# tommybazar/TBRaymarcherPlugin

Hardware: AMD Instinct MI355X
Metric: volume Msamples/s (rays x steps) at 512^3, 1024^2 view; % HBM roofline (higher is better)
Workload: dtype f32

## Files before the change

tbraymarcherplugin_amd/csrc/tbrm_api.cpp:

```cpp
#include "tbrm_resources.h"
#include "tbrm_light_sweep.h"

#include <algorithm>
#include <atomic>
#include <cctype>
#include <cmath>
#include <cstdarg>
#include <cstdio>
#include <climits>
#include <cstdlib>
#include <cstring>
#include <new>
#include <vector>

using namespace tbrm;
using namespace tbrm_host;

namespace {
thread_local char g_error[512] = "";

struct TunableDef { const char* name; int def; };
const TunableDef kTunables[TUNE_COUNT] = {
    {"force_slice_kernel", 0}, {"chunk_steps", 0}, {"occ_slices", 0}, {"sparse_occ", 1}, {"occ_list", 1}, {"light_cache_mb", -1},
    {"light_batching", 1}, {"share_grid", 1}, {"ray_wave_skip", -1}, {"ray_lanes", 0}, {"chain_fast_loop", 1},
    {"chain_rect_planes", 1}, {"occ_overlap", 2}, {"light_sweep", 1}, {"sweep_prefetch", 0}, {"stream_priority", 0}, {"sweep_debug", 0},
    {"sweep_timeout_ms", 0}, {"fast_window_div", 1}, {"slab_sweep", 0}, {"gpu_timing", 1}, {"ray_tables", 1}, {"sweep_epoch_preset", 0}, {"occ_dual", 1}, {"sweep_chain", 4}, {"ray_xcd_rows", 1},
    {"ray_labels", 0}, {"stats_groups", 0}, {"occ_run", 4}, {"view_cache_mb", 1536},
};
struct TunableStore {
    std::atomic<int> v[TUNE_COUNT];
    TunableStore()
    {
        for (int t = 0; t < TUNE_COUNT; ++t) {
            char env[64] = "TBRM_";
            size_t n = strlen(env);
            for (const char* c = kTunables[t].name; *c && n + 1 < sizeof(env); ++c) env[n++] = (char) toupper((unsigned char) *c);
            env[n] = 0;
            const char* e = getenv(env);
            v[t].store(e && *e ? atoi(e) : kTunables[t].def, std::memory_order_relaxed);
        }
    }
};
TunableStore g_tunables;
}

namespace tbrm {
int tune(Tunable t) { return g_tunables.v[t].load(std::memory_order_relaxed); }
}

int tbrm_set_tunable(const char* name, int32_t value)
{
    if (!name) return tbrm_host::fail(TBRM_ERR_INVALID_ARG, "null argument");
    for (int t = 0; t < TUNE_COUNT; ++t)
        if (!strcmp(name, kTunables[t].name)) { g_tunables.v[t].store(value, std::memory_order_relaxed); return TBRM_OK; }
    return tbrm_host::fail(TBRM_ERR_INVALID_ARG, "no tunable named '%s'", name);
}

int tbrm_get_tunable(const char* name, int32_t* value)
{
    if (!name || !value) return tbrm_host::fail(TBRM_ERR_INVALID_ARG, "null argument");
    for (int t = 0; t < TUNE_COUNT; ++t)
        if (!strcmp(name, kTunables[t].name)) { *value = tune((Tunable) t); return TBRM_OK; }
    return tbrm_host::fail(TBRM_ERR_INVALID_ARG, "no tunable named '%s'", name);
}

namespace tbrm_host {

int fail(int code, const char* fmt, ...)
{
    va_list ap;
    va_start(ap, fmt);
    vsnprintf(g_error, sizeof(g_error), fmt, ap);
    va_end(ap);
    return code;
}

int bind(const tbrm_resources* r)
{
    HIP_TRY(hipSetDevice(r->desc.device));
    return TBRM_OK;
}

bool initialized(const tbrm_resources* r) { return r && r->has_volume && r->has_tf && r->d_light; }

VolumeDev data_view(const tbrm_resources* r)
{
    const tbrm_resources::Residency& q = r->res_data;
    return VolumeDev{r->d_data, r->desc.dim_x, r->desc.dim_y, r->desc.dim_z, r->desc.data_format, r->dbn[0], r->dbn[0] * r->dbn[1],
                     q.wrap_src, (q.hi - q.wrap_src) * 8};
}
static void window_division(float center, float width, float* inv_width, int* fast_div)
{
    *inv_width = 0.0f;
    *fast_div = 0;
    if (tune(TUNE_FAST_WINDOW_DIV) == 0 || !std::isfinite(center) || !std::isfinite(width)) return;
    const float aw = std::fabs(width), ac = std::fabs(center);
    if (!(aw >= 0x1p-40f && aw <= 0x1p40f) || ac > 0x1p40f) return;
    uint32_t bits;
    memcpy(&bits, &width, 4);
    if ((bits & 0x007fffffu) == 0x007fffffu) return;
    *inv_width = 1.0f / width;
    *fast_div = 1;
}

WindowDev window_dev_of(float center, float width, int low_cutoff, int high_cutoff)
{
    WindowDev w{center, width, low_cutoff ? 1.0f : 0.0f, high_cutoff ? 1.0f : 0.0f, 0.0f, 0};
    window_division(center, width, &w.inv_width, &w.fast_div);
    return w;
}
// ... 750 lines not shown
```

tbraymarcherplugin_amd/csrc/tbrm_api_render.cpp:

```cpp
#include "tbrm_resources.h"
#include "../../include/tbrm_view_cache.h"

#include <algorithm>
#include <cmath>
#include <cstdio>
#include <cstring>
#include <vector>

using namespace tbrm;
using namespace tbrm_host;

namespace {

int build_ray_params(tbrm_resources* r, const tbrm_camera* cam, const tbrm_tile* tile, const tbrm_raymarch_params* rp,
                     const tbrm_world_params* world, RayParams& p)
{
    if (!(rp->steps > 0.0f)) return fail(TBRM_ERR_INVALID_ARG, "steps must be > 0");
    if (tile->w < 0 || tile->h < 0 || cam->width <= 0 || cam->height <= 0) return fail(TBRM_ERR_INVALID_ARG, "bad tile/camera size");
    std::memset(&p, 0, sizeof(p));
    p.data = data_view(r);
    p.data_addr_mode = r->desc.data_address_mode == TBRM_ADDRESS_CLAMP ? ADDR_CLAMP : ADDR_WRAP;
    p.tf = r->d_tf;
    p.win = window_dev(r);
    p.xcd_rows = tune(TUNE_RAY_XCD_ROWS);
    p.light = r->d_light;
    for (int c = 0; c < 3; ++c) p.lv_dims[c] = r->lv_dims[c];
    p.lv_bnx = r->lbn[0];
    p.lv_bnxy = r->lbn[0] * r->lbn[1];
    p.lv_fmt = r->lv_fmt;
    p.lv_wrap_layer = r->res_light.wrap_src;
    p.lv_wrap_shift = (r->res_light.hi - r->res_light.wrap_src) * 8;
    const tbrm_vec3d* v[4] = {&cam->position, &cam->forward, &cam->right, &cam->up};
    float* dst[4] = {p.cam_pos, p.fwd, p.right, p.up};
    for (int k = 0; k < 4; ++k) {
        dst[k][0] = (float) v[k]->x; dst[k][1] = (float) v[k]->y; dst[k][2] = (float) v[k]->z;
    }
    p.thx = (float) cam->tan_half_fov_x;
    p.thy = (float) cam->tan_half_fov_y;
    p.width = cam->width;
    p.height = cam->height;
    host_world_to_local(world->volume_transform, p.m);
    host_local_clipping(*world, p.cc, p.cd);
    p.clip_mode = raymarch_clip_mode(p.cc, p.cd);
    {
        const int ws = tune(TUNE_RAY_WAVE_SKIP);
        p.wave_skip = ws > 0 || (ws < 0 && std::min(r->desc.dim_x, std::min(r->desc.dim_y, r->desc.dim_z)) >= 384) ? 1 : 0;
    }
    p.share_grid = (r->lv_dims[0] == r->desc.dim_x && r->lv_dims[1] == r->desc.dim_y && r->lv_dims[2] == r->desc.dim_z &&
                    !r->resident && tune(TUNE_SHARE_GRID)) ? 1 : 0;
    p.tile_x0 = tile->x0; p.tile_y0 = tile->y0; p.tile_w = tile->w; p.tile_h = tile->h;
    p.row_group_step = tile->row_group_step > 0 ? tile->row_group_step : 1;
    p.steps = rp->steps;
    p.jitter_frame = rp->jitter_frame;
    p.bnx = r->bn[0]; p.bny = r->bn[1]; p.bnz = r->bn[2];
    p.tab = r->d_ray_tab;
    return TBRM_OK;
}

int attach_skipping(tbrm_resources* r, const tbrm_raymarch_params* rp, RayParams& p)
{
    if (!rp->enable_skipping) return TBRM_OK;
    if (int e = ensure_skipping(r)) return e;
    p.empty_bits = r->d_empty;
    p.skip_dist = r->d_dist[0];
    return TBRM_OK;
}

template <class March> int deliver_frame(tbrm_resources* r, const tbrm_tile* tile, float* host_out_rgba, March&& march, bool* delivered = nullptr)
{
    if (!r || !tile || !host_out_rgba) return fail(TBRM_ERR_INVALID_ARG, "null argument");
    if (tile->w < 0 || tile->h < 0) return fail(TBRM_ERR_INVALID_ARG, "bad tile size");
    const size_t bytes = (size_t) tile->w * tile->h * 4 * sizeof(float);
    if (bytes == 0) return TBRM_OK;
    if (int e = bind(r)) return e;
    if (bytes > r->out_bytes) {
        HIP_TRY(hipStreamSynchronize(r->stream));
        (void) hipFree(r->d_out);
        r->d_out = nullptr;
        r->out_bytes = 0;
        HIP_TRY(hipMalloc((void**) &r->d_out, bytes));
        r->out_bytes = bytes;
    }
    if (int e = march(r->d_out)) return e;
    HIP_TRY(hipMemcpyAsync(host_out_rgba, r->d_out, bytes, hipMemcpyDeviceToHost, r->stream));
    HIP_TRY(hipStreamSynchronize(r->stream));
    if (delivered) *delivered = true;
    return TBRM_OK;
}


bool carve_view_arena(ViewCache& v, const RayParams& p)
{
    const size_t bw = 8, bh = v.lanes == 4 ? 8 : 4;
    const size_t waves = ((size_t) p.tile_w + bw - 1) / bw * (((size_t) p.tile_h + bh - 1) / bh) * 4;
    const size_t align = 256, header = (2 * waves * sizeof(uint32_t) + 16 + align - 1) / align * align;
    if (!v.arena || waves > 0xffffffffu || header + 2 * align + kRayRecordTripBytes > v.arena_bytes) return false;
    const size_t cap = std::min<size_t>((v.arena_bytes - header - align) / kRayRecordTripBytes, 0xffffffffu);
    v.n_waves = (uint32_t) waves;
    v.cap_trips = (uint32_t) cap;
    v.rec.counts = reinterpret_cast<uint32_t*>(v.arena);
    v.rec.offsets = v.rec.counts + waves;
    v.rec.meta = v.rec.offsets + waves;
    v.rec.base = reinterpret_cast<int32_t*>(v.arena + header);
    v.rec.rows = v.arena + header + (cap * sizeof(int32_t) + align - 1) / align * align;
    return true;
}

int march_or_relight(tbrm_resources* r, RayParams& p)
{
    ViewCache& v = r->view;
    const auto plain = [&]() -> int {
        HIP_TRY(launch_raymarch(p, r->stream));
        ++v.stats[0];
        return TBRM_OK;
    };
    if (tune(TUNE_VIEW_CACHE_MB) <= 0 || p.depth || r->d_labels || p.slab_on || r->resident || p.tile_w <= 0 || p.tile_h <= 0) {
        v.state = ViewCache::kNone;
        v.stats[5] = 0;
        return plain();
    }
    RayParams key;
    std::memcpy(&key, &p, sizeof(key));
    key.out = nullptr;
    const int lanes = ray_lanes_for(p), tables = ray_tables_for(p) ? 1 : 0;
    if (v.state == ViewCache::kNone || v.lanes != lanes || v.tables != tables || v.data_gen != r->data_gen || v.tf_gen != r->tf_gen ||
        std::memcmp(&v.key, &key, sizeof(key)) != 0) {
        std::memcpy(&v.key, &key, sizeof(key));
        v.lanes = lanes;
        v.tables = tables;
        v.data_gen = r->data_gen;
        v.tf_gen = r->tf_gen;
        v.state = ViewCache::kPlain;
        v.stats[5] = 0;
        return plain();
    }
    switch (v.state) {
    case ViewCache::kPlain:
        ensure_view_arena(r, false);
        if (!carve_view_arena(v, p)) {
            v.state = ViewCache::kTooLarge;
            ++v.stats[4];
            return plain();
        }
        p.rec = v.rec;
        HIP_TRY(launch_raymarch_recording(p, false, r->stream));
        v.state = ViewCache::kCounted;
        ++v.stats[1];
        return TBRM_OK;
    case ViewCache::kCounted:
        p.rec = v.rec;
        HIP_TRY(launch_view_scan(v.rec, v.n_waves, v.cap_trips, r->stream));
        HIP_TRY(launch_raymarch_recording(p, true, r->stream));
        HIP_TRY(hipMemcpyAsync(v.meta_host, v.rec.meta, 2 * sizeof(uint32_t), hipMemcpyDeviceToHost, r->stream));
        HIP_TRY(hipEventRecord(v.ev_meta, r->stream));
        v.state = ViewCache::kFilled;
        ++v.stats[2];
        return TBRM_OK;
    case ViewCache::kFilled: {
        const hipError_t q = hipEventQuery(v.ev_meta);
        if (q == hipErrorNotReady) {
            (void) hipGetLastError();
            return plain();
        }
        HIP_TRY(q);
        if (!v.meta_host[1]) {
            v.state = ViewCache::kTooLarge;
            ++v.stats[4];
            return plain();
        }
        v.state = ViewCache::kReady;
        v.stats[5] = (uint64_t) v.meta_host[0] * kRayRecordTripBytes + 2 * (uint64_t) v.n_waves * sizeof(uint32_t);
        [[fallthrough]];
    }
    case ViewCache::kReady:
        p.rec = v.rec;
        HIP_TRY(launch_relight(p, r->stream));
        ++v.stats[3];
        return TBRM_OK;
    default:
        return plain();
    }
}

}

namespace tbrm_host {

void ensure_view_arena(tbrm_resources* r, bool eager)
{
    ViewCache& v = r->view;
    const int mb = tune(TUNE_VIEW_CACHE_MB);
    if (v.arena_tried || mb <= 0 || r->resident || r->light_channels != 1) return;
    v.arena_tried = true;
    size_t want = (size_t) mb << 20, free_b = 0, total_b = 0;
    if (hipMemGetInfo(&free_b, &total_b) == hipSuccess) {
        const size_t spare = free_b > ((size_t) 8 << 30) ? free_b - ((size_t) 8 << 30) : 0;
        want = std::min(want, eager ? spare / 2 : spare / 8);
    } else (void) hipGetLastError();
    void* a = nullptr;
    void* h = nullptr;
    hipEvent_t ev = nullptr;
    if (want >= ((size_t) 64 << 10) && hipMalloc(&a, want) == hipSuccess && hipHostMalloc(&h, 4 * sizeof(uint32_t), hipHostMallocDefault) == hipSuccess &&
        hipEventCreateWithFlags(&ev, hipEventDisableTiming) == hipSuccess) {
        v.arena = (char*) a;
        v.arena_bytes = want;
        v.meta_host = (uint32_t*) h;
        v.ev_meta = ev;
        return;
    }
    (void) hipGetLastError();
    if (a) (void) hipFree(a);
    if (h) (void) hipHostFree(h);
}

void release_view_cache(tbrm_resources* r)
{
    ViewCache& v = r->view;
    if (v.arena) (void) hipFree(v.arena);
    if (v.meta_host) (void) hipHostFree(v.meta_host);
    if (v.ev_meta) (void) hipEventDestroy(v.ev_meta);
    v = ViewCache{};
}

}

extern "C" {

int tbrm_view_cache_abi_version(void) { return TBRM_VIEW_CACHE_ABI_VERSION; }

int tbrm_view_cache_stats(const tbrm_resources* r, uint64_t out[6])
{
    if (!r || !out) return fail(TBRM_ERR_INVALID_ARG, "null argument");
    for (int k = 0; k < 6; ++k) out[k] = r->view.stats[k];
    return TBRM_OK;
}

int tbrm_raymarch_lit_device(tbrm_resources* r, const tbrm_camera* cam, const tbrm_tile* tile, const tbrm_raymarch_params* rp,
                             const tbrm_world_params* world, const float* device_scene_depth, float* device_out_rgba)
{
    if (r && r->resident) return fail(TBRM_ERR_UNSUPPORTED, "slab-resident handle: frames are marched with tbrm_raymarch_lit_slab_device");
    if (!r || !cam || !tile || !rp || !world || !device_out_rgba) return fail(TBRM_ERR_INVALID_ARG, "null argument");
    if (!initialized(r)) return fail(TBRM_ERR_NOT_INITIALIZED, "resources have no volume or transfer function");
    if (int e = bind(r)) return e;
    RayParams p;
    if (int e = build_ray_params(r, cam, tile, rp, world, p)) return e;
    p.depth = device_scene_depth;
    p.out = device_out_rgba;
    if (int e = attach_skipping(r, rp, p)) return e;
    if (int e = label_ray_params(r, p)) return e;
    if (int e = begin_timed(r, 1)) return e;
    if (r->light_channels == 3) {
        p.light = r->light_channel(0);
        p.light_g = r->light_channel(1);
        p.light_b = r->light_channel(2);
        HIP_TRY(launch_raymarch_rgb(p, r->stream));
    } else if (int e = march_or_relight(r, p)) return e;
    ++r->launches[2];
    return end_timed(r, 1);
}
// ... 151 lines not shown
```

tbraymarcherplugin_amd/csrc/tbrm_internal.h:

```cpp
#pragma once
#include <hip/hip_runtime.h>
#include <stdint.h>

namespace tbrm {

enum : int { FMT_U8 = 0, FMT_U16 = 1, FMT_F32 = 2 };
enum : int { ADDR_WRAP = 0, ADDR_CLAMP = 1, ADDR_BORDER = 2 };

enum : int { PASS_ADD = 0, PASS_CHANGE = 1, PASS_ADD2 = 2, PASS_CHANGE_ONE = 3, PASS_PLANES = 5 };

constexpr int kBrick = 8;
constexpr int kBrickShift = 3;

struct VolumeDev {
    const void* data;
    int nx, ny, nz;
    int fmt;
    int bnx;
    int bnxy;
    int wrap_layer;
    int wrap_shift;
};

struct WindowDev {
// ... 75 lines not shown
    const uint8_t* occ_flags;
    int occ_phase;
    uint8_t* occ_flags_out;
    int occ_blocks_x, occ_blocks_y, occ_groups;
    int pass_start, pass_slices, chunk_slices;
    const uint32_t* occ_list;
    const int* occ_count;
    int occ_grid_cap;
    uint32_t* occ_list_out;
    int* occ_count_out;
    int* occ_count_host;
    int32_t* occ_slot_out;
    int compact;
    const float* ones;
    ChunkStream a, r;
};

struct DualPass {
    int axis, start, dir;
    int blocks_x, blocks_y;
    float step100[2];
    float* fs_keep[2];
    float* fs_spill[2];
    uint32_t fs_cap[2];
    const int32_t* fs_slot;
    const uint8_t* flags;
};
struct DualOcc {
    int on;
    DualPass pass[2];
};
constexpr int kOccRunMax = 64;
constexpr int kRunLenShift = 26;
constexpr uint32_t kRunNone = 0xffffffffu;
constexpr size_t kRunMaskWords = 4096;
struct OccRuns {
    int len;
    uint32_t* list;
    int* count;
    int* count_host;
};
struct SweepParams {
    int sx, sy;
    int hx, hy;
    int r_from_records;
    int r_sx, r_sy, r_hx, r_hy;
    uint32_t r_epoch;
    uint32_t* rec[2];
    uint32_t epoch;
    int unused0;
    int stagger_ns;
    int* ticket;
    int debug;
    unsigned long long* stamps;
    int unused1;
    int lv_f32;
    int reinit_slice;
    int n_real;
    int* error;
    unsigned long long give_up_ticks;
};

struct SweepLink {
    uint32_t* prog_out;
    const uint32_t* prog_in;
    uint32_t in_epoch;
    int in_axis, in_tiles_x;
    int in_down, in_layer0, in_G;
    int coherent_loads;
    int ticket0;
    int total_tiles;
};
constexpr int kSweepChainMax = 4;
struct SweepChainPass {
    ChunkParams p;
    SweepParams q;
    SweepLink link;
};
struct SweepChainArgs {
    int n;
    SweepChainPass pass[kSweepChainMax];
};

constexpr size_t kRayRecordRowBytes = 64 * (sizeof(float4) + 3 * sizeof(float));
constexpr size_t kRayRecordTripBytes = kRayRecordRowBytes + sizeof(int32_t);
struct RayRecord {
    uint32_t* counts;
    uint32_t* offsets;
    uint32_t* meta;
    int32_t* base;
    char* rows;
};

struct RayParams {
    VolumeDev data;
    int data_addr_mode;
    const float4* tf;
    WindowDev win;
    const void* light;
    int lv_dims[3];
    int lv_bnx, lv_bnxy;
    int lv_fmt;
    float cam_pos[3], fwd[3], right[3], up[3];
    float thx, thy;
    int width, height;
    float m[12];
    float cc[3], cd[3];
    int clip_mode;
    int share_grid;
    int wave_skip;
    int tile_x0, tile_y0, tile_w, tile_h, row_group_step;
    float steps;
    int jitter_frame;
    const float* depth;
    float* out;
    const uint32_t* empty_bits;
    int xcd_rows;
    const uint2* tab;
    const uint8_t* skip_dist;
    int bnx, bny, bnz;
    unsigned long long* sample_counter;
    int lv_wrap_layer, lv_wrap_shift;
    int slab_on, slab_z0, slab_z1, slab_dir;
    const uint16_t* octree;
    int oct_dims[3];
    float oct_depth0;
    const uint8_t* labels;
    const float4* lab_colors;
    const void* light_g;
    const void* light_b;
    RayRecord rec;
};

int ray_lanes_for(const RayParams& p);
bool ray_tables_for(const RayParams& p);

constexpr int kRayTabApron = 2;
constexpr int ray_tab_axis_entries(int n) { return n + 2 * kRayTabApron; }
constexpr int ray_tab_index(int texel) { return texel + kRayTabApron; }
constexpr int ray_tab_last_base(int n) { return ray_tab_axis_entries(n) - 2; }
constexpr int ray_tab_entries(int nx, int ny, int nz) { return (ray_tab_axis_entries(nx) + ray_tab_axis_entries(ny) + ray_tab_axis_entries(nz) + 1) & ~1; }

struct BrickParams {
    VolumeDev data;
    int addr_mode;
    int bnx, bny, bnz;
    float2* minmax;
    int bz0, bz1;
};

struct EmptyParams {
    const float2* minmax;
    int n_bricks;
    WindowDev win;
    const int* alpha_prefix;
    uint32_t* bits;
};

hipError_t launch_shell_transparent(const EmptyParams& p, int bnx, int bny, int bnz, float border, int* flag, hipStream_t s);

constexpr int kSkipDistCap = 32;
struct DistParams {
    const uint32_t* bits;
    const uint8_t* in;
    uint8_t* out;
    int bn[3];
    int axis;
};

struct OctreeParams {
    VolumeDev data;
    const uint16_t* lower;
    int lower_dims[3];
    uint16_t* out;
    int dims[3];
};

struct RelayoutParams {
    const void* src;
    void* dst;
    int nx, ny, nz;
    int bnx, bnxy, bnz;
    int elem_bytes;
    int to_bricks;
};

constexpr int kOccSlices = 8;
constexpr int kChunkTile = 32;
constexpr int kChunkThreads = 1024;
constexpr int kChunkMaxHull = 64;

enum Tunable : int {
    TUNE_FORCE_SLICE_KERNEL,
    TUNE_CHUNK_STEPS,
    TUNE_OCC_SLICES,
    TUNE_SPARSE_OCC,
    TUNE_OCC_LIST,
    TUNE_LIGHT_CACHE_MB,
    TUNE_LIGHT_BATCHING,
    TUNE_SHARE_GRID,
    TUNE_RAY_WAVE_SKIP,
    TUNE_RAY_LANES,
    TUNE_CHAIN_FAST_LOOP,
    TUNE_CHAIN_RECT_PLANES,
    TUNE_OCC_OVERLAP,
    TUNE_LIGHT_SWEEP,
    TUNE_SWEEP_PREFETCH,
    TUNE_STREAM_PRIORITY,
    TUNE_SWEEP_DEBUG,
    TUNE_SWEEP_TIMEOUT_MS,
    TUNE_FAST_WINDOW_DIV,
    TUNE_SLAB_SWEEP,
    TUNE_GPU_TIMING,
    TUNE_RAY_TABLES,
    TUNE_SWEEP_EPOCH_PRESET,
    TUNE_OCC_DUAL,
    TUNE_SWEEP_CHAIN,
    TUNE_RAY_XCD_ROWS,
    TUNE_RAY_LABELS,
    TUNE_STATS_GROUPS,
    TUNE_OCC_RUN,
    TUNE_VIEW_CACHE_MB,
    TUNE_COUNT
};
int tune(Tunable t);

hipError_t launch_selftest_decode(float* d_u8, float* d_u16, hipStream_t s);
hipError_t launch_selftest_roundtrip(const float* d_in, float* d_out, size_t n, hipStream_t s);
hipError_t launch_selftest_window_division(const WindowDev& w, unsigned long long* d_mismatches, hipStream_t s);
hipError_t launch_selftest_opacity_correction(float step0, float step1, unsigned long long* d_mismatches, hipStream_t s);
hipError_t launch_relayout(const RelayoutParams& p, hipStream_t s);
size_t chunk_lds_bytes(const ChunkParams& p, int mode, int lv_fmt);
size_t occlusion_lds_bytes(const ChunkParams& p);
constexpr int kPlaneGuard = 4096;
hipError_t launch_occ_flags(const ChunkParams& p, int mode, int n_chunks, hipStream_t s);
hipError_t launch_light_occlusion(const ChunkParams& p, int mode, hipStream_t s, const DualOcc* dual = nullptr, const OccRuns* runs = nullptr);
hipError_t launch_unit_flags(const ChunkParams& pc, const DualOcc& d, hipStream_t s);
bool occ_runs_apply(const ChunkParams& pc);
hipError_t launch_occ_runs(const ChunkParams& pc, const OccRuns& runs, hipStream_t s);
hipError_t launch_light_chain(const ChunkParams& p, int mode, int lv_fmt, hipStream_t s);
hipError_t launch_light_sweep(const ChunkParams& p, const SweepParams& q, int mode, hipStream_t s);
hipError_t launch_light_sweep_chain(const SweepChainArgs& c, int mode, hipStream_t s);
hipError_t launch_fill(void* dst, int fmt, size_t n, float value, hipStream_t s);
hipError_t launch_propagate_slice(const PropParams& p, bool change, hipStream_t s);
hipError_t launch_raymarch(const RayParams& p, hipStream_t s);
hipError_t launch_raymarch_rgb(const RayParams& p, hipStream_t s);
hipError_t launch_raymarch_recording(const RayParams& p, bool fill, hipStream_t s);
hipError_t launch_view_scan(const RayRecord& rec, uint32_t n_waves, uint32_t cap_trips, hipStream_t s);
hipError_t launch_relight(const RayParams& p, hipStream_t s);
hipError_t launch_raymarch_intensity(const RayParams& p, hipStream_t s);
hipError_t launch_raymarch_octree(const RayParams& p, hipStream_t s);
hipError_t launch_octree_level(const OctreeParams& p, bool base, hipStream_t s);
hipError_t launch_count_samples(const RayParams& p, hipStream_t s);
hipError_t launch_brick_minmax(const BrickParams& p, hipStream_t s);
hipError_t launch_brick_empty(const EmptyParams& p, hipStream_t s);
hipError_t launch_brick_dist(const DistParams& p, int addr_mode, hipStream_t s);

struct LabelBrickParams {
    const uint8_t* labels;
    uint32_t* masks;
    int bnx, bny;
    int b0[3], b1[3];
};
struct LabelLiveParams {
    const uint32_t* masks;
    int n_bricks;
    uint32_t alive[8];
    uint32_t* live;
    uint32_t* present;
};
struct LabelMergeParams {
    const uint32_t* empty;
    const uint32_t* live;
    uint32_t* out;
    int bn[3];
};
struct LabelRegionParams {
    const uint8_t* src;
    uint8_t* dst;
    int origin[3], extent[3];
    int bnx, bnxy;
};
hipError_t launch_label_brick_masks(const LabelBrickParams& p, hipStream_t s);
hipError_t launch_label_live(const LabelLiveParams& p, hipStream_t s);
hipError_t launch_label_merge(const LabelMergeParams& p, int addr_mode, hipStream_t s);
hipError_t launch_label_region(const LabelRegionParams& p, hipStream_t s);

struct VolumeRegionParams {
    const void* box;
    void* bricked;
    int origin[3], extent[3];
    int bnx, bnxy;
    int elem_bytes;
    int to_bricks;
};
struct BrickReach {
    int lo[3], hi[3], last[3];
    int n[3];
};
hipError_t launch_volume_region(const VolumeRegionParams& p, hipStream_t s);
hipError_t launch_brick_minmax_region(const BrickParams& p, const BrickReach& q, hipStream_t s);

constexpr int kStatsMaxBins = 4096;
constexpr int kStatsLabelWords = 256 * 6;
struct StatsParams {
    const void* data;
    const uint8_t* labels;
    int fmt;
    int bnx, bnxy;
    int origin[3], end[3];
    int b0[3], nb[3];
    uint32_t n_bins;
    uint32_t lo_code, hi_code;
    uint32_t div_mul, div_shift;
    float lo_f, hi_f, scale;
    uint32_t copies;
    uint32_t mask[8];
    uint32_t* out;
};
hipError_t launch_volume_histogram(const StatsParams& p, bool masked, int grid, hipStream_t s);
hipError_t launch_label_statistics(const StatsParams& p, int grid, hipStream_t s);

}
```

tbraymarcherplugin_amd/csrc/tbrm_kernels.hip:

```cpp
#include "tbrm_device_sampling.h"

#include <algorithm>
#include <type_traits>

namespace tbrm {

#if defined(TBRM_RAY_RGB_UNIT) || defined(TBRM_RAY_REC_UNIT)
#define TBRM_RAY_ONLY_UNIT 1
#undef TBRM_RAY_STATS
#endif
#ifndef TBRM_RAY_ONLY_UNIT

template <int FMT>
__global__ void k_fill(void* dst, size_t n, float value)
{
    const size_t stride = (size_t) gridDim.x * blockDim.x;
    for (size_t i = (size_t) blockIdx.x * blockDim.x + threadIdx.x; i < n; i += stride) store_voxel<FMT>(dst, i, value);
}

hipError_t launch_fill(void* dst, int fmt, size_t n, float value, hipStream_t s)
{
    if (n == 0) return hipSuccess;
    if (fmt == FMT_U8) {
        float x = value;
// ... 301 lines not shown
                if constexpr (TAB) dist = p.skip_dist[tab_brick];
                else {
                    const int bx = address<DMODE>(ix, p.data.nx) >> kBrickShift;
                    const int by = address<DMODE>(iy, p.data.ny) >> kBrickShift;
                    const int bz = address<DMODE>(iz, p.data.nz) >> kBrickShift;
                    dist = p.skip_dist[(bz * p.bny + by) * p.bnx + bx];
                }
                live = live && dist == 0;
                if (dist >= 2) safe_until = max(safe_until, idx + (int) fminf(((float) (8 * (dist - 1)) - 1.25f) * inv_texels_per_step, 1.0e6f));
            }
        }
        const bool any_live = !wave_skip || __builtin_amdgcn_ballot_w64(live) != 0;
#ifdef TBRM_RAY_STATS
        {
            const unsigned long long nd = __builtin_popcountll(__builtin_amdgcn_ballot_w64(!done)), nl = __builtin_popcountll(__builtin_amdgcn_ballot_w64(live));
            if (lane == 0) { atomicAdd(&g_ray_stats[0], 1ull); atomicAdd(&g_ray_stats[1], nd); atomicAdd(&g_ray_stats[2], nl); if (nl) atomicAdd(&g_ray_stats[3], 1ull); }
        }
#endif
        if (live) {
            RawTaps<DFMT> dtaps;
            RawTaps<LFMT> ltaps;
            [[maybe_unused]] TapOffsets lt{};
            float gx, gy, gz;
            TapOffsets dt;
            if constexpr (TAB) dt = tab_dt;
            else dt = tap_offsets<DMODE, SLAB>(p.data, ix, iy, iz);
            dtaps.issue(p.data.data, dt);
            if constexpr (LABELS) {
                const int lx = (int) __builtin_rintf((float) (p.data.nx - 1) * saturate_(q0));
                const int ly = (int) __builtin_rintf((float) (p.data.ny - 1) * saturate_(q1));
                const int lz = (int) __builtin_rintf((float) (p.data.nz - 1) * saturate_(q2));
                lab = p.labels[brick_off(lx, ly, lz, p.data.bnx, p.data.bnxy)];
            }
            const float sp0 = saturate_(q0), sp1 = saturate_(q1), sp2 = saturate_(q2);
            if (same_grid && sp0 == q0 && sp1 == q1 && sp2 == q2) {
                gx = fx; gy = fy; gz = fz;
                if constexpr (RGB) lt = dt;
                else ltaps.issue(p.light, dt);
            } else {
                int lx, ly, lz;
                texel_split_bounded(sp0, lnx, lx, gx);
                texel_split_bounded(sp1, lny, ly, gy);
                texel_split_bounded(sp2, lnz, lz, gz);
                if constexpr (RGB) lt = tap_offsets<ADDR_WRAP, SLAB>(lightv, lx, ly, lz);
                else ltaps.issue(p.light, tap_offsets<ADDR_WRAP, SLAB>(lightv, lx, ly, lz));
            }
            const float v = dtaps.filter(fx, fy, fz);
            const float tpos = window_position<DFMT != FMT_F32>(v, p.win);
            if (!((tpos < 0.0f && p.win.low_cutoff > 0.0f) || (tpos > 1.0f && p.win.high_cutoff > 0.0f))) {
                const float4 cs = sample_tf(s_tf, tpos);
                const float a_sat = saturate_(cs.w);
                if (a_sat != 0.0f) {
                    const float a = one_minus_pow01_(1.0f - a_sat, step);
                    if constexpr (RGB) {
                        ltaps.issue(p.light, lt);
                        const float lr = ltaps.filter(gx, gy, gz);
                        ltaps.issue(p.light_g, lt);
                        const float lg = ltaps.filter(gx, gy, gz);
                        ltaps.issue(p.light_b, lt);
                        const float lb = ltaps.filter(gx, gy, gz);
                        x = make_float4((cs.x * lr) * a, (cs.y * lg) * a, (cs.z * lb) * a, a);
                    } else {
                        const float l = ltaps.filter(gx, gy, gz);
                        x = make_float4((cs.x * l) * a, (cs.y * l) * a, (cs.z * l) * a, a);
                        if constexpr (REC == REC_FILL) { rec_x = make_float4(cs.x, cs.y, cs.z, a); rec_sp0 = sp0; rec_sp1 = sp1; rec_sp2 = sp2; }
                    }
                }
            }
            if constexpr (LABELS) {
                if (is_full && s_lab[lab].w == 0.0f) lab = -1;
            }
        }

        bool to_accumulate = x.w >= 0.0f || x.w != x.w;
        if constexpr (LABELS) to_accumulate = to_accumulate || lab >= 0;
        const bool any_x = __builtin_amdgcn_ballot_w64(to_accumulate) != 0;
#ifdef TBRM_RAY_STATS
        {
            const unsigned long long nx = __builtin_popcountll(__builtin_amdgcn_ballot_w64(x.w >= 0.0f || x.w != x.w));
            if (lane == 0 && nx) { atomicAdd(&g_ray_stats[4], 1ull); atomicAdd(&g_ray_stats[5], nx); }
        }
#endif
        if (any_x) {
            if constexpr (REC == REC_FILL) {
                if (n_rec < rec_room) {
                    const size_t trip = (size_t) rec_first + n_rec;
                    char* const row = p.rec.rows + trip * kRayRecordRowBytes;
                    if (lane == 0) p.rec.base[trip] = base;
                    reinterpret_cast<float4*>(row)[lane] = rec_x;
                    float* const sp = reinterpret_cast<float*>(row + 64 * sizeof(float4));
                    sp[lane] = rec_sp0; sp[64 + lane] = rec_sp1; sp[128 + lane] = rec_sp2;
                }
            }
            if constexpr (REC != REC_OFF) ++n_rec;
#include "tbrm_ray_replay.inc"
        }
        if (base + kRayLanes >= n_samples) done = true;
        const bool renewed = eager;
        eager = false;
        if (!any_live) {
            int k_lane = INT32_MAX;
            if (!done) {
                const int ahead = safe_until - base - b;
                const int by_safe = ahead >= kRayLanes ? ahead / kRayLanes : 0;
                const int left = max_steps - 1 - (base + kRayLanes);
                const int by_length = left >= kRayLanes ? left / kRayLanes : 0;
                k_lane = min(by_safe, by_length);
            }
            int k = 0;
            while (k < 64 && __builtin_amdgcn_ballot_w64(k_lane <= k) == 0) ++k;
            if (k > 0) {
                for (int t = 0; t < k * kRayLanes; ++t) { pos0 = pos0 + sv0; pos1 = pos1 + sv1; pos2 = pos2 + sv2; }
                adds += k * kRayLanes;
                base += k * kRayLanes;
            }
            if (renewed && k == 0) renew_wait = 4;
            else if (renew_wait > 0) --renew_wait;
            eager = renew_wait == 0;
        }
    }
    if ((SLAB ? mine : valid) && b == 0) reinterpret_cast<float4*>(p.out)[(size_t) j * p.tile_w + i] = make_float4(le[0], le[1], le[2], le[3]);
    if constexpr (REC == REC_COUNT) {
        if (lane == 0) p.rec.counts[ray_wave_number()] = n_rec;
    }
}

template <int RL> static dim3 ray_grid(const RayParams& p)
{
    constexpr int BW = 8, BH = RL == 4 ? 8 : 4;
    return dim3((p.tile_w + BW - 1) / BW, (p.tile_h + BH - 1) / BH);
}
template <int DFMT, int LFMT, int RL, bool SLAB, bool TAB, bool LABELS, bool RGB, int REC>
static hipError_t launch_lit(const RayParams& p, size_t lds_bytes, hipStream_t s)
{
    const dim3 grid = ray_grid<RL>(p), block(256);
    if (p.data_addr_mode == ADDR_CLAMP) hipLaunchKernelGGL((k_raymarch_lit<DFMT, LFMT, ADDR_CLAMP, RL, SLAB, TAB, LABELS, RGB, REC>), grid, block, lds_bytes, s, p);
    else hipLaunchKernelGGL((k_raymarch_lit<DFMT, LFMT, ADDR_WRAP, RL, SLAB, TAB, LABELS, RGB, REC>), grid, block, lds_bytes, s, p);
    return hipGetLastError();
}
#ifndef TBRM_RAY_ONLY_UNIT
bool ray_tables_for(const RayParams& p)
{
    const size_t tab_bytes = (size_t) ray_tab_entries(p.data.nx, p.data.ny, p.data.nz) * sizeof(uint2);
    return !p.slab_on && p.tab != nullptr && tune(TUNE_RAY_TABLES) != 0 && (float) std::max(p.data.nx, std::max(p.data.ny, p.data.nz)) <= p.steps && tab_bytes <= 16 * 1024;
}
#endif
template <int DFMT, int LFMT, int RL, bool LABELS, bool RGB, int REC>
static hipError_t launch_ray3(const RayParams& p, hipStream_t s)
{
    constexpr size_t lab_bytes = LABELS ? 256 * sizeof(float4) + 256 * sizeof(short) : 0;
    if (p.slab_on) {
        if constexpr (LABELS || RGB || REC != REC_OFF) return hipErrorInvalidValue;
        else return launch_lit<DFMT, LFMT, RL, true, false, false, false, REC_OFF>(p, 0, s);
    }
    const size_t tab_bytes = (size_t) ray_tab_entries(p.data.nx, p.data.ny, p.data.nz) * sizeof(uint2);
    if (ray_tables_for(p)) return launch_lit<DFMT, LFMT, RL, false, true, LABELS, RGB, REC>(p, tab_bytes + lab_bytes, s);
    return launch_lit<DFMT, LFMT, RL, false, false, LABELS, RGB, REC>(p, lab_bytes, s);
}
#ifndef TBRM_RAY_ONLY_UNIT
int ray_lanes_for(const RayParams& p)
{
    const double load = (double) p.tile_w * (double) p.tile_h * 512.0 / (double) (p.steps > 1.0f ? p.steps : 1.0f);
    const int forced = tune(TUNE_RAY_LANES);
    return (forced ? forced : (load <= 700000.0 ? 8 : 4)) == 8 ? 8 : 4;
}
#endif
template <int DFMT, int LFMT, bool RGB, int REC>
static hipError_t launch_ray2(const RayParams& p, hipStream_t s)
{
    const int rl = ray_lanes_for(p);
    if constexpr (RGB) {
        if (p.labels || !p.light_g || !p.light_b) return hipErrorInvalidValue;
        return rl == 8 ? launch_ray3<DFMT, LFMT, 8, false, true, REC>(p, s) : launch_ray3<DFMT, LFMT, 4, false, true, REC>(p, s);
    } else if constexpr (REC != REC_OFF) {
        if (p.labels) return hipErrorInvalidValue;
        return rl == 8 ? launch_ray3<DFMT, LFMT, 8, false, false, REC>(p, s) : launch_ray3<DFMT, LFMT, 4, false, false, REC>(p, s);
    } else {
        if (p.labels) return rl == 8 ? launch_ray3<DFMT, LFMT, 8, true, false, REC>(p, s) : launch_ray3<DFMT, LFMT, 4, true, false, REC>(p, s);
        return rl == 8 ? launch_ray3<DFMT, LFMT, 8, false, false, REC>(p, s) : launch_ray3<DFMT, LFMT, 4, false, false, REC>(p, s);
    }
}
template <int DFMT, bool RGB, int REC>
static hipError_t launch_ray1(const RayParams& p, hipStream_t s)
{
    return p.lv_fmt == FMT_U8 ? launch_ray2<DFMT, FMT_U8, RGB, REC>(p, s) : launch_ray2<DFMT, FMT_F32, RGB, REC>(p, s);
}
template <bool RGB, int REC = REC_OFF>
static hipError_t launch_ray0(const RayParams& p, hipStream_t s)
{
    if (p.tile_w <= 0 || p.tile_h <= 0) return hipSuccess;
    switch (p.data.fmt) {
        case FMT_U8: return launch_ray1<FMT_U8, RGB, REC>(p, s);
        case FMT_U16: return launch_ray1<FMT_U16, RGB, REC>(p, s);
        default: return launch_ray1<FMT_F32, RGB, REC>(p, s);
    }
}
#if defined(TBRM_RAY_RGB_UNIT)
hipError_t launch_raymarch_rgb(const RayParams& p, hipStream_t s) { return launch_ray0<true>(p, s); }
#elif defined(TBRM_RAY_REC_UNIT)
hipError_t launch_raymarch_recording(const RayParams& p, bool fill, hipStream_t s)
{
    return fill ? launch_ray0<false, REC_FILL>(p, s) : launch_ray0<false, REC_COUNT>(p, s);
}

__global__ __launch_bounds__(1024) void k_view_scan(const RayRecord rec, uint32_t n_waves, uint32_t cap_trips)
{
    __shared__ unsigned long long s_sum[1024];
    const uint32_t per = (n_waves + 1023u) / 1024u;
    const uint32_t w0 = (uint32_t) min((unsigned long long) threadIdx.x * per, (unsigned long long) n_waves), w1 = (uint32_t) min((unsigned long long) w0 + per, (unsigned long long) n_waves);
    unsigned long long sum = 0;
    for (uint32_t w = w0; w < w1; ++w) sum += rec.counts[w];
    s_sum[threadIdx.x] = sum;
    __syncthreads();
    for (int d = 1; d < 1024; d <<= 1) {
        const unsigned long long v = (int) threadIdx.x >= d ? s_sum[threadIdx.x - d] : 0ull;
        __syncthreads();
        s_sum[threadIdx.x] += v;
        __syncthreads();
    }
    unsigned long long at = s_sum[threadIdx.x] - sum;
    for (uint32_t w = w0; w < w1; ++w) { rec.offsets[w] = (uint32_t) at; at += rec.counts[w]; }
    if (threadIdx.x == 1023) {
        const unsigned long long total = s_sum[1023];
        rec.meta[0] = (uint32_t) min(total, 0xffffffffull);
        rec.meta[1] = total <= cap_trips ? 1u : 0u;
    }
}
hipError_t launch_view_scan(const RayRecord& rec, uint32_t n_waves, uint32_t cap_trips, hipStream_t s)
{
    hipLaunchKernelGGL(k_view_scan, dim3(1), dim3(1024), 0, s, rec, n_waves, cap_trips);
    return hipGetLastError();
}

struct RelightTrip { int base; float4 c; float sp0, sp1, sp2; };
__device__ __forceinline__ RelightTrip relight_load(const RayRecord& rec, size_t trip, int lane)
{
    const char* const row = rec.rows + trip * kRayRecordRowBytes;
    const float* const sp = reinterpret_cast<const float*>(row + 64 * sizeof(float4));
    return RelightTrip{rec.base[trip], reinterpret_cast<const float4*>(row)[lane], sp[lane], sp[64 + lane], sp[128 + lane]};
}
template <int LFMT, int kRayLanes>
__global__ __launch_bounds__(256) void k_relight(const RayParams p)
{
    constexpr int LSH = kRayLanes == 4 ? 2 : 3;
    __shared__ float4 s_x[256];
    const int lane = threadIdx.x & 63, wave = threadIdx.x >> 6;
    const int b = lane & (kRayLanes - 1), r = lane >> LSH;
    int i, j, px, py;
    ray_of_wave<kRayLanes>(p, wave, r, i, j);
    const bool valid = tile_pixel_at(p, i, j, px, py);
    Ray ray;
    cube_setup(p, valid ? px : p.tile_x0, valid ? py : p.tile_y0, ray);
    const March m = march_setup(p, ray, px, py, valid);
    const int max_steps = m.max_steps, n_samples = m.n_samples;

    const float lnx = (float) p.lv_dims[0], lny = (float) p.lv_dims[1], lnz = (float) p.lv_dims[2];
    const VolumeDev lightv{p.light, p.lv_dims[0], p.lv_dims[1], p.lv_dims[2], LFMT, p.lv_bnx, p.lv_bnxy, p.lv_wrap_layer, p.lv_wrap_shift};
    float le[4] = {0.0f, 0.0f, 0.0f, 0.0f};
    bool done = n_samples == 0;
    float4* const xs = s_x + (threadIdx.x & ~(kRayLanes - 1));
    constexpr bool LABELS = false;
    [[maybe_unused]] short* const s_lb = nullptr;
    [[maybe_unused]] const float4* const s_lab = nullptr;
    [[maybe_unused]] const int lab = -1;
    [[maybe_unused]] const float final_step = 0.0f;

    const uint32_t w = ray_wave_number();
    const uint32_t n = p.rec.counts[w];
    const size_t first = p.rec.offsets[w];
    RelightTrip next{};
    if (n > 0) next = relight_load(p.rec, first, lane);
    for (uint32_t trip = 0; trip < n; ++trip) {
        const RelightTrip cur = next;
        if (trip + 1 < n) next = relight_load(p.rec, first + trip + 1, lane);
        float4 x = make_float4(0.0f, 0.0f, 0.0f, -1.0f);
        if (cur.c.w >= 0.0f || cur.c.w != cur.c.w) {
            int lx, ly, lz;
            float gx, gy, gz;
            texel_split_bounded(cur.sp0, lnx, lx, gx);
            texel_split_bounded(cur.sp1, lny, ly, gy);
            texel_split_bounded(cur.sp2, lnz, lz, gz);
            RawTaps<LFMT> ltaps;
            ltaps.issue(p.light, tap_offsets<ADDR_WRAP, false>(lightv, lx, ly, lz));
            const float l = ltaps.filter(gx, gy, gz);
            x = make_float4((cur.c.x * l) * cur.c.w, (cur.c.y * l) * cur.c.w, (cur.c.z * l) * cur.c.w, cur.c.w);
        }
        const int base = cur.base;
        {
#include "tbrm_ray_replay.inc"
        }
        if (base + kRayLanes >= n_samples) done = true;
    }
    if (valid && b == 0) reinterpret_cast<float4*>(p.out)[(size_t) j * p.tile_w + i] = make_float4(le[0], le[1], le[2], le[3]);
}
template <int LFMT, int RL> static hipError_t launch_relight2(const RayParams& p, hipStream_t s)
{
    hipLaunchKernelGGL((k_relight<LFMT, RL>), ray_grid<RL>(p), dim3(256), 0, s, p);
    return hipGetLastError();
}
hipError_t launch_relight(const RayParams& p, hipStream_t s)
{
    if (p.tile_w <= 0 || p.tile_h <= 0) return hipSuccess;
    const bool eight = ray_lanes_for(p) == 8;
    if (p.lv_fmt == FMT_U8) return eight ? launch_relight2<FMT_U8, 8>(p, s) : launch_relight2<FMT_U8, 4>(p, s);
    return eight ? launch_relight2<FMT_F32, 8>(p, s) : launch_relight2<FMT_F32, 4>(p, s);
}
#else
hipError_t launch_raymarch(const RayParams& p, hipStream_t s) { return launch_ray0<false>(p, s); }

__global__ __launch_bounds__(256) void k_selftest_window_division(WindowDev w, unsigned long long* mismatches)
{
    const uint32_t last = 0x3f800000u;
    unsigned long long bad = 0;
    for (uint64_t i = (uint64_t) blockIdx.x * blockDim.x + threadIdx.x; i <= last; i += (uint64_t) gridDim.x * blockDim.x) {
        const float v = __uint_as_float((uint32_t) i);
        const float a = tf_position(v, w.center, w.width), b = tf_position_fast(v, w.center, w.width, w.inv_width);
        if (__float_as_uint(a) != __float_as_uint(b)) ++bad;
    }
    if (bad) atomicAdd(mismatches, bad);
}
hipError_t launch_selftest_window_division(const WindowDev& w, unsigned long long* d_mismatches, hipStream_t s)
{
    hipLaunchKernelGGL(k_selftest_window_division, dim3(256 * 64), dim3(256), 0, s, w, d_mismatches);
    return hipGetLastError();
}

__global__ __launch_bounds__(256) void k_selftest_opacity_correction(float step0, float step1, unsigned long long* mismatches)
{
    const uint32_t last = 0x3f800000u;
    unsigned long long bad = 0;
    for (uint64_t i = (uint64_t) blockIdx.x * blockDim.x + threadIdx.x; i <= last; i += (uint64_t) gridDim.x * blockDim.x) {
        const float x = __uint_as_float((uint32_t) i);
        float p0, p1, s0, s1;
        pow01_2_(x, step0, step1, p0, p1);
        one_minus_pow01_2_(x, step0, step1, s0, s1);
        const float a = 1.0f - pow01_(x, step0), b = one_minus_pow01_(x, step0);
        if (__float_as_uint(1.0f - p0) != __float_as_uint(s0) || __float_as_uint(1.0f - p1) != __float_as_uint(s1) || __float_as_uint(a) != __float_as_uint(b)) ++bad;
    }
    if (bad) atomicAdd(mismatches, bad);
}
hipError_t launch_selftest_opacity_correction(float step0, float step1, unsigned long long* d_mismatches, hipStream_t s)
{
    hipLaunchKernelGGL(k_selftest_opacity_correction, dim3(256 * 64), dim3(256), 0, s, step0, step1, d_mismatches);
    return hipGetLastError();
}

static hipError_t launch_pixel_blocks(void (*kernel)(const RayParams), const RayParams& p, hipStream_t s)
{
    if (p.tile_w <= 0 || p.tile_h <= 0) return hipSuccess;
    hipLaunchKernelGGL(kernel, dim3((p.tile_w + 15) / 16, (p.tile_h + 15) / 16), dim3(256), 0, s, p);
    return hipGetLastError();
}

template <int DFMT>
__global__ __launch_bounds__(256) void k_raymarch_intensity(const RayParams p)
{
    int i, j, px, py;
    if (!tile_pixel(p, i, j, px, py)) return;
    Ray ray;
    cube_setup(p, px, py, ray);
    const March m = march_setup(p, ray, px, py, true);
    const float sv0 = m.sv[0], sv1 = m.sv[1], sv2 = m.sv[2];
    float pos0 = m.pos[0], pos1 = m.pos[1], pos2 = m.pos[2];
    const float nx = (float) p.data.nx, ny = (float) p.data.ny, nz = (float) p.data.nz;
    auto intensity = [&](float u, float v, float w) -> float {
        int ix, iy, iz;
        float fx, fy, fz;
        texel_split(u, nx, ix, fx);
        texel_split(v, ny, iy, fy);
        texel_split(w, nz, iz, fz);
        const float val = sample_trilinear_at<DFMT>(p.data.data, tap_offsets<ADDR_CLAMP>(p.data, ix, iy, iz), fx, fy, fz);
        return __builtin_amdgcn_fmed3f(tf_position(val, p.win.center, p.win.width), 0.0f, 1.0f);
    };
    float4 out = make_float4(0.0f, 0.0f, 0.0f, 0.0f);
    bool hit = false;
    for (int k = 0; k < m.max_steps; ++k) {
        pos0 = pos0 + sv0; pos1 = pos1 + sv1; pos2 = pos2 + sv2;
        const float s0 = saturate_(pos0), s1 = saturate_(pos1), s2 = saturate_(pos2);
        if (!(p.clip_mode && is_clipped(s0, s1, s2, p.cc, p.cd))) {
            const float t = intensity(s0, s1, s2);
            out = make_float4(t, t, t, 1.0f);
            hit = true;
            break;
        }
    }
    if (!hit && m.final_step > 0.0f) {
        pos0 = pos0 + (sv0 * m.final_step); pos1 = pos1 + (sv1 * m.final_step); pos2 = pos2 + (sv2 * m.final_step);
        if (!(p.clip_mode && is_clipped(pos0, pos1, pos2, p.cc, p.cd))) {
// ... 113 lines not shown
```

tbraymarcherplugin_amd/csrc/tbrm_ray_replay.inc:

```
            s_x[threadIdx.x] = x;
            if constexpr (LABELS) s_lb[threadIdx.x] = (short) lab;
            __builtin_amdgcn_wave_barrier();
#pragma unroll
            for (int t = 0; t < kRayLanes; ++t) {
                const float4 c = xs[t];
                const bool is_full_step = base + t < max_steps;
                const bool data_step = !(c.w < 0.0f);
                if (done || (!LABELS && !data_step)) continue;
                if (data_step) accumulate(le, c);
                if constexpr (LABELS) {
                    const int lb = s_lb[(threadIdx.x & ~(kRayLanes - 1)) + t];
                    if (lb >= 0) {
                        float4 e;
                        if (is_full_step) e = s_lab[lb];
                        else {
                            const float4 raw = p.lab_colors[lb];
                            const float a = raw.w != 0.0f ? one_minus_pow01_(1.0f - raw.w, 100.0f * final_step) : 0.0f;
                            e = make_float4(raw.x * a, raw.y * a, raw.z * a, a);
                        }
                        accumulate(le, e);
                    }
                }
                if (exit_reached(le[3], is_full_step)) { le[3] = 1.0f; done = true; }
            }
            __builtin_amdgcn_wave_barrier();
```

Baseline: 108,400.

## Record per-sample transmittance so relight replays as independent weighted sums

During the recording pass, each lane now stores the transmittance (1-alpha) in front of its sample, plus the final per-ray alpha. The relight kernel then no longer redoes ray setup or the serial front-to-back compositing through shared memory. Each trip contributes an independent weighted term, summed across lanes with DPP, and trips are unrolled with depth U to overlap light-volume gathers. The record layout changes to two float4 rows per trip, and the base array is dropped. This relies on the recorded opacities staying unchanged between fill and relight, and the transmittance capture sits behind a TBRM_RAY_REC_UNIT macro.

```diff
diff --git a/tbraymarcherplugin_amd/csrc/tbrm_api.cpp b/tbraymarcherplugin_amd/csrc/tbrm_api.cpp
--- a/tbraymarcherplugin_amd/csrc/tbrm_api.cpp
+++ b/tbraymarcherplugin_amd/csrc/tbrm_api.cpp
@@ -25,7 +25,7 @@
     {"light_batching", 1}, {"share_grid", 1}, {"ray_wave_skip", -1}, {"ray_lanes", 0}, {"chain_fast_loop", 1},
     {"chain_rect_planes", 1}, {"occ_overlap", 2}, {"light_sweep", 1}, {"sweep_prefetch", 0}, {"stream_priority", 0}, {"sweep_debug", 0},
     {"sweep_timeout_ms", 0}, {"fast_window_div", 1}, {"slab_sweep", 0}, {"gpu_timing", 1}, {"ray_tables", 1}, {"sweep_epoch_preset", 0}, {"occ_dual", 1}, {"sweep_chain", 4}, {"ray_xcd_rows", 1},
-    {"ray_labels", 0}, {"stats_groups", 0}, {"occ_run", 4}, {"view_cache_mb", 1536},
+    {"ray_labels", 0}, {"stats_groups", 0}, {"occ_run", 4}, {"view_cache_mb", 1536}, {"relight_depth", 0},
 };
 struct TunableStore {
     std::atomic<int> v[TUNE_COUNT];
diff --git a/tbraymarcherplugin_amd/csrc/tbrm_api_render.cpp b/tbraymarcherplugin_amd/csrc/tbrm_api_render.cpp
--- a/tbraymarcherplugin_amd/csrc/tbrm_api_render.cpp
+++ b/tbraymarcherplugin_amd/csrc/tbrm_api_render.cpp
@@ -93,16 +93,17 @@
 {
     const size_t bw = 8, bh = v.lanes == 4 ? 8 : 4;
     const size_t waves = ((size_t) p.tile_w + bw - 1) / bw * (((size_t) p.tile_h + bh - 1) / bh) * 4;
-    const size_t align = 256, header = (2 * waves * sizeof(uint32_t) + 16 + align - 1) / align * align;
-    if (!v.arena || waves > 0xffffffffu || header + 2 * align + kRayRecordTripBytes > v.arena_bytes) return false;
-    const size_t cap = std::min<size_t>((v.arena_bytes - header - align) / kRayRecordTripBytes, 0xffffffffu);
+    const size_t align = 256, words = (2 * waves * sizeof(uint32_t) + 16 + align - 1) / align * align;
+    const size_t header = words + (waves * (64 / v.lanes) * sizeof(float) + align - 1) / align * align;
+    if (!v.arena || waves > 0xffffffffu || header + kRayRecordTripBytes > v.arena_bytes) return false;
+    const size_t cap = std::min<size_t>((v.arena_bytes - header) / kRayRecordTripBytes, 0xffffffffu);
     v.n_waves = (uint32_t) waves;
     v.cap_trips = (uint32_t) cap;
     v.rec.counts = reinterpret_cast<uint32_t*>(v.arena);
     v.rec.offsets = v.rec.counts + waves;
     v.rec.meta = v.rec.offsets + waves;
-    v.rec.base = reinterpret_cast<int32_t*>(v.arena + header);
-    v.rec.rows = v.arena + header + (cap * sizeof(int32_t) + align - 1) / align * align;
+    v.rec.alpha = reinterpret_cast<float*>(v.arena + words);
+    v.rec.rows = v.arena + header;
     return true;
 }
 
@@ -169,12 +170,12 @@
             return plain();
         }
         v.state = ViewCache::kReady;
-        v.stats[5] = (uint64_t) v.meta_host[0] * kRayRecordTripBytes + 2 * (uint64_t) v.n_waves * sizeof(uint32_t);
+        v.stats[5] = (uint64_t) v.meta_host[0] * kRayRecordTripBytes + (uint64_t) v.n_waves * ray_record_wave_bytes(v.lanes);
         [[fallthrough]];
     }
     case ViewCache::kReady:
         p.rec = v.rec;
-        HIP_TRY(launch_relight(p, r->stream));
+        HIP_TRY(launch_relight(p, relight_depth_for(v.meta_host[0], v.n_waves), r->stream));
         ++v.stats[3];
         return TBRM_OK;
     default:
diff --git a/tbraymarcherplugin_amd/csrc/tbrm_internal.h b/tbraymarcherplugin_amd/csrc/tbrm_internal.h
--- a/tbraymarcherplugin_amd/csrc/tbrm_internal.h
+++ b/tbraymarcherplugin_amd/csrc/tbrm_internal.h
@@ -181,13 +181,14 @@
     SweepChainPass pass[kSweepChainMax];
 };
 
-constexpr size_t kRayRecordRowBytes = 64 * (sizeof(float4) + 3 * sizeof(float));
-constexpr size_t kRayRecordTripBytes = kRayRecordRowBytes + sizeof(int32_t);
+constexpr size_t kRayRecordRowBytes = 64 * sizeof(float4);
+constexpr size_t kRayRecordTripBytes = 2 * kRayRecordRowBytes;
+constexpr size_t ray_record_wave_bytes(int ray_lanes) { return 2 * sizeof(uint32_t) + (size_t) (64 / ray_lanes) * sizeof(float); }
 struct RayRecord {
     uint32_t* counts;
     uint32_t* offsets;
     uint32_t* meta;
-    int32_t* base;
+    float* alpha;
     char* rows;
 };
 
@@ -320,6 +321,7 @@
     TUNE_STATS_GROUPS,
     TUNE_OCC_RUN,
     TUNE_VIEW_CACHE_MB,
+    TUNE_RELIGHT_DEPTH,
     TUNE_COUNT
 };
 int tune(Tunable t);
@@ -346,7 +348,8 @@
 hipError_t launch_raymarch_rgb(const RayParams& p, hipStream_t s);
 hipError_t launch_raymarch_recording(const RayParams& p, bool fill, hipStream_t s);
 hipError_t launch_view_scan(const RayRecord& rec, uint32_t n_waves, uint32_t cap_trips, hipStream_t s);
-hipError_t launch_relight(const RayParams& p, hipStream_t s);
+int relight_depth_for(uint64_t trips, uint32_t waves);
+hipError_t launch_relight(const RayParams& p, int depth, hipStream_t s);
 hipError_t launch_raymarch_intensity(const RayParams& p, hipStream_t s);
 hipError_t launch_raymarch_octree(const RayParams& p, hipStream_t s);
 hipError_t launch_octree_level(const OctreeParams& p, bool base, hipStream_t s);
diff --git a/tbraymarcherplugin_amd/csrc/tbrm_kernels.hip b/tbraymarcherplugin_amd/csrc/tbrm_kernels.hip
--- a/tbraymarcherplugin_amd/csrc/tbrm_kernels.hip
+++ b/tbraymarcherplugin_amd/csrc/tbrm_kernels.hip
@@ -407,18 +407,16 @@
         }
 #endif
         if (any_x) {
+            [[maybe_unused]] float rec_om = -1.0f;
+#include "tbrm_ray_replay.inc"
             if constexpr (REC == REC_FILL) {
                 if (n_rec < rec_room) {
-                    const size_t trip = (size_t) rec_first + n_rec;
-                    char* const row = p.rec.rows + trip * kRayRecordRowBytes;
-                    if (lane == 0) p.rec.base[trip] = base;
-                    reinterpret_cast<float4*>(row)[lane] = rec_x;
-                    float* const sp = reinterpret_cast<float*>(row + 64 * sizeof(float4));
-                    sp[lane] = rec_sp0; sp[64 + lane] = rec_sp1; sp[128 + lane] = rec_sp2;
+                    float4* const rows = reinterpret_cast<float4*>(p.rec.rows + ((size_t) rec_first + n_rec) * kRayRecordTripBytes);
+                    rows[lane] = rec_x;
+                    rows[64 + lane] = make_float4(rec_sp0, rec_sp1, rec_sp2, rec_om);
                 }
             }
             if constexpr (REC != REC_OFF) ++n_rec;
-#include "tbrm_ray_replay.inc"
         }
         if (base + kRayLanes >= n_samples) done = true;
         const bool renewed = eager;
@@ -447,6 +445,9 @@
     if ((SLAB ? mine : valid) && b == 0) reinterpret_cast<float4*>(p.out)[(size_t) j * p.tile_w + i] = make_float4(le[0], le[1], le[2], le[3]);
     if constexpr (REC == REC_COUNT) {
         if (lane == 0) p.rec.counts[ray_wave_number()] = n_rec;
+    }
+    if constexpr (REC == REC_FILL) {
+        if (b == 0) p.rec.alpha[(size_t) ray_wave_number() * (64 / kRayLanes) + r] = le[3];
     }
 }
 
@@ -557,78 +558,106 @@
     return hipGetLastError();
 }
 
-struct RelightTrip { int base; float4 c; float sp0, sp1, sp2; };
-__device__ __forceinline__ RelightTrip relight_load(const RayRecord& rec, size_t trip, int lane)
-{
-    const char* const row = rec.rows + trip * kRayRecordRowBytes;
-    const float* const sp = reinterpret_cast<const float*>(row + 64 * sizeof(float4));
-    return RelightTrip{rec.base[trip], reinterpret_cast<const float4*>(row)[lane], sp[lane], sp[64 + lane], sp[128 + lane]};
-}
-template <int LFMT, int kRayLanes>
+struct RelightTrip { float4 a, b; };
+template <int U>
+__device__ __forceinline__ void relight_load(RelightTrip (&rec)[U], const float4* rows, uint32_t trip, uint32_t n)
+{
+#pragma unroll
+    for (int u = 0; u < U; ++u) {
+        rec[u].a = make_float4(0.0f, 0.0f, 0.0f, 0.0f);
+        rec[u].b = make_float4(0.0f, 0.0f, 0.0f, -1.0f);
+        if (trip + u < n) {
+            rec[u].a = rows[(size_t) (trip + u) * 128];
+            rec[u].b = rows[(size_t) (trip + u) * 128 + 64];
+        }
+    }
+}
+template <int T> __device__ __forceinline__ float relight_from_lane_ahead(float v)
+{
+    if constexpr (T == 0) return v;
+    else return __int_as_float(__builtin_amdgcn_update_dpp(0, __float_as_int(v), 0x100 + T , 0xf, 0xf, true));
+}
+template <int T, int kRayLanes>
+__device__ __forceinline__ void relight_add(float (&le)[3], float t0, float t1, float t2)
+{
+    if constexpr (T < kRayLanes) {
+        le[0] = le[0] + relight_from_lane_ahead<T>(t0);
+        le[1] = le[1] + relight_from_lane_ahead<T>(t1);
+        le[2] = le[2] + relight_from_lane_ahead<T>(t2);
+        relight_add<T + 1, kRayLanes>(le, t0, t1, t2);
+    }
+}
+template <int LFMT, int kRayLanes, int U>
 __global__ __launch_bounds__(256) void k_relight(const RayParams p)
 {
     constexpr int LSH = kRayLanes == 4 ? 2 : 3;
-    __shared__ float4 s_x[256];
     const int lane = threadIdx.x & 63, wave = threadIdx.x >> 6;
     const int b = lane & (kRayLanes - 1), r = lane >> LSH;
     int i, j, px, py;
     ray_of_wave<kRayLanes>(p, wave, r, i, j);
     const bool valid = tile_pixel_at(p, i, j, px, py);
-    Ray ray;
-    cube_setup(p, valid ? px : p.tile_x0, valid ? py : p.tile_y0, ray);
-    const March m = march_setup(p, ray, px, py, valid);
-    const int max_steps = m.max_steps, n_samples = m.n_samples;
 
     const float lnx = (float) p.lv_dims[0], lny = (float) p.lv_dims[1], lnz = (float) p.lv_dims[2];
     const VolumeDev lightv{p.light, p.lv_dims[0], p.lv_dims[1], p.lv_dims[2], LFMT, p.lv_bnx, p.lv_bnxy, p.lv_wrap_layer, p.lv_wrap_shift};
-    float le[4] = {0.0f, 0.0f, 0.0f, 0.0f};
-    bool done = n_samples == 0;
-    float4* const xs = s_x + (threadIdx.x & ~(kRayLanes - 1));
-    constexpr bool LABELS = false;
-    [[maybe_unused]] short* const s_lb = nullptr;
-    [[maybe_unused]] const float4* const s_lab = nullptr;
-    [[maybe_unused]] const int lab = -1;
-    [[maybe_unused]] const float final_step = 0.0f;
-
     const uint32_t w = ray_wave_number();
-    const uint32_t n = p.rec.counts[w];
-    const size_t first = p.rec.offsets[w];
-    RelightTrip next{};
-    if (n > 0) next = relight_load(p.rec, first, lane);
-    for (uint32_t trip = 0; trip < n; ++trip) {
-        const RelightTrip cur = next;
-        if (trip + 1 < n) next = relight_load(p.rec, first + trip + 1, lane);
-        float4 x = make_float4(0.0f, 0.0f, 0.0f, -1.0f);
-        if (cur.c.w >= 0.0f || cur.c.w != cur.c.w) {
-            int lx, ly, lz;
-            float gx, gy, gz;
-            texel_split_bounded(cur.sp0, lnx, lx, gx);
-            texel_split_bounded(cur.sp1, lny, ly, gy);
-            texel_split_bounded(cur.sp2, lnz, lz, gz);
-            RawTaps<LFMT> ltaps;
-            ltaps.issue(p.light, tap_offsets<ADDR_WRAP, false>(lightv, lx, ly, lz));
-            const float l = ltaps.filter(gx, gy, gz);
-            x = make_float4((cur.c.x * l) * cur.c.w, (cur.c.y * l) * cur.c.w, (cur.c.z * l) * cur.c.w, cur.c.w);
-        }
-        const int base = cur.base;
-        {
-#include "tbrm_ray_replay.inc"
-        }
-        if (base + kRayLanes >= n_samples) done = true;
-    }
-    if (valid && b == 0) reinterpret_cast<float4*>(p.out)[(size_t) j * p.tile_w + i] = make_float4(le[0], le[1], le[2], le[3]);
-}
-template <int LFMT, int RL> static hipError_t launch_relight2(const RayParams& p, hipStream_t s)
-{
-    hipLaunchKernelGGL((k_relight<LFMT, RL>), ray_grid<RL>(p), dim3(256), 0, s, p);
+    const uint32_t n = __builtin_amdgcn_readfirstlane(p.rec.counts[w]);
+    const float4* const rows = reinterpret_cast<const float4*>(p.rec.rows + (size_t) __builtin_amdgcn_readfirstlane(p.rec.offsets[w]) * kRayRecordTripBytes) + lane;
+    const float alpha = p.rec.alpha[(size_t) w * (64 / kRayLanes) + r];
+
+    float le[3] = {0.0f, 0.0f, 0.0f};
+    RelightTrip cur[U];
+    relight_load(cur, rows, 0, n);
+    for (uint32_t trip = 0; trip < n; trip += U) {
+        RawTaps<LFMT> taps[U];
+        float gx[U], gy[U], gz[U];
+#pragma unroll
+        for (int u = 0; u < U; ++u) {
+            if (!(cur[u].b.w < 0.0f)) {
+                int lx, ly, lz;
+                texel_split_bounded(cur[u].b.x, lnx, lx, gx[u]);
+                texel_split_bounded(cur[u].b.y, lny, ly, gy[u]);
+                texel_split_bounded(cur[u].b.z, lnz, lz, gz[u]);
+                taps[u].issue(p.light, tap_offsets<ADDR_WRAP, false>(lightv, lx, ly, lz));
+            }
+        }
+        RelightTrip next[U];
+        relight_load(next, rows, trip + U, n);
+#pragma unroll
+        for (int u = 0; u < U; ++u) {
+            float t0 = 0.0f, t1 = 0.0f, t2 = 0.0f;
+            if (!(cur[u].b.w < 0.0f)) {
+                const float l = taps[u].filter(gx[u], gy[u], gz[u]);
+                const float4 c = cur[u].a;
+                const float om = cur[u].b.w;
+                t0 = ((c.x * l) * c.w) * om;
+                t1 = ((c.y * l) * c.w) * om;
+                t2 = ((c.z * l) * c.w) * om;
+            }
+            relight_add<0, kRayLanes>(le, t0, t1, t2);
+            cur[u] = next[u];
+        }
+    }
+    if (valid && b == 0) reinterpret_cast<float4*>(p.out)[(size_t) j * p.tile_w + i] = make_float4(le[0], le[1], le[2], alpha);
+}
+template <int LFMT, int RL> static hipError_t launch_relight2(const RayParams& p, int depth, hipStream_t s)
+{
+    if (depth == 4) hipLaunchKernelGGL((k_relight<LFMT, RL, 4>), ray_grid<RL>(p), dim3(256), 0, s, p);
+    else if (depth == 2) hipLaunchKernelGGL((k_relight<LFMT, RL, 2>), ray_grid<RL>(p), dim3(256), 0, s, p);
+    else hipLaunchKernelGGL((k_relight<LFMT, RL, 1>), ray_grid<RL>(p), dim3(256), 0, s, p);
     return hipGetLastError();
 }
-hipError_t launch_relight(const RayParams& p, hipStream_t s)
+int relight_depth_for(uint64_t trips, uint32_t waves)
+{
+    const int forced = tune(TUNE_RELIGHT_DEPTH);
+    if (forced) return forced >= 4 ? 4 : (forced >= 2 ? 2 : 1);
+    return trips >= 4 * (uint64_t) waves ? 4 : 1;
+}
+hipError_t launch_relight(const RayParams& p, int depth, hipStream_t s)
 {
     if (p.tile_w <= 0 || p.tile_h <= 0) return hipSuccess;
     const bool eight = ray_lanes_for(p) == 8;
-    if (p.lv_fmt == FMT_U8) return eight ? launch_relight2<FMT_U8, 8>(p, s) : launch_relight2<FMT_U8, 4>(p, s);
-    return eight ? launch_relight2<FMT_F32, 8>(p, s) : launch_relight2<FMT_F32, 4>(p, s);
+    if (p.lv_fmt == FMT_U8) return eight ? launch_relight2<FMT_U8, 8>(p, depth, s) : launch_relight2<FMT_U8, 4>(p, depth, s);
+    return eight ? launch_relight2<FMT_F32, 8>(p, depth, s) : launch_relight2<FMT_F32, 4>(p, depth, s);
 }
 #else
 hipError_t launch_raymarch(const RayParams& p, hipStream_t s) { return launch_ray0<false>(p, s); }
diff --git a/tbraymarcherplugin_amd/csrc/tbrm_ray_replay.inc b/tbraymarcherplugin_amd/csrc/tbrm_ray_replay.inc
--- a/tbraymarcherplugin_amd/csrc/tbrm_ray_replay.inc
+++ b/tbraymarcherplugin_amd/csrc/tbrm_ray_replay.inc
@@ -6,6 +6,11 @@
                 const float4 c = xs[t];
                 const bool is_full_step = base + t < max_steps;
                 const bool data_step = !(c.w < 0.0f);
+#ifdef TBRM_RAY_REC_UNIT
+                if constexpr (REC == REC_FILL) {
+                    if (t == b && !done && data_step) rec_om = 1.0f - le[3];
+                }
+#endif
                 if (done || (!LABELS && !data_step)) continue;
                 if (data_step) accumulate(le, c);
                 if constexpr (LABELS) {
```

Result: slower. 103,600 (-4.4%).
